# davidfischinger/haf_grasping

Measured on AMD Instinct MI355X. Metric: grid-cell x rotation SVM evals/sec, higher is better.
Workload: dtype f16

## Files before the change

haf_grasping_amd/build.py:

```python
import os
import re
import subprocess
import sys

HERE = os.path.dirname(os.path.abspath(__file__))
CSRC = os.path.join(HERE, "csrc")
LIB = os.path.join(HERE, "libhafgrasp.so")
LIB_TESTING = os.path.join(HERE, "libhafgrasp_testing.so")
ENGINE_SOURCES = ["engine.cpp", "engine_tables.cpp", "engine_request.cpp", "engine_geometry.cpp", "engine_debug.cpp", "engine_topgrasps.cpp"]
TESTING_ONLY = ["engine_testing.cpp", "testkernels.hip"]
SOURCES = ["prestages.hip", "features.hip", "contraction.hip", "screen.hip", "recheck.hip", "exact8.hip", "vote.hip", "prob.hip", "topgrasps.hip"] + \
          ENGINE_SOURCES + ["parsers.cpp", "multi.cpp"]
EXTRA = {"screen.hip": ["-fno-slp-vectorize"]}
HEADERS = ["kernels.h", "device_common.h", "feature_device.h", "screen_band.h", "parsers.h", "decq.h", "engine_internal.h", "engine_state.h"] + TESTING_ONLY + [ os.path.join("..", "..", "include", "hafgrasp.h"),
           os.path.join("..", "cli", "haf_grasp_cli.cpp"), os.path.join("..", "..", "ros_shim", "shim_core.h")]
FLAGS = ["--offload-arch=gfx950", "-O3", "-std=c++17", "-fPIC", "-ffp-contract=off", "-fno-fast-math",
         "-Wall", "-Wno-unused-result", "-Wno-inline-asm"]
ROCM = os.environ.get("ROCM_PATH", "/opt/rocm")
OBJDUMP = os.path.join(ROCM, "lib", "llvm", "bin", "llvm-objdump")
EXP_HAZARD_KERNELS = ["k_svm_screen", "k_svm_rbf_h", "k_svm_rbf"]
EXP_MIN_DISTANCE = 8


def up_to_date():
# ... 117 lines not shown
    for line in text.splitlines():
        m = re.match(r"^[0-9a-f]+ <(\S+)>:", line)
        if m:
            cur = m.group(1) if (DESCRIPTOR_LOAD_KERNELS in m.group(1) and not m.group(1).endswith(".kd")) else None
            if cur:
                rep[cur] = 0
            continue
        if cur and line.split("//")[0].strip().startswith(("global_load", "buffer_load")):
            rep[cur] += 1
    return rep


def check_descriptor_loads(lib=None, verbose=False):
    rep = descriptor_load_report(lib)
    if verbose:
        for k, n in sorted(rep.items()):
            print("  descriptor-load check: %-60s %3d vector loads" % (k[:60], n))
    if not rep:
        raise RuntimeError("check_descriptor_loads: no %s instance found in %s" % (DESCRIPTOR_LOAD_KERNELS, lib or LIB))
    bad = {k: n for k, n in rep.items() if n > MAX_VECTOR_LOADS}
    if bad:
        raise RuntimeError("build check failed: the group-parallel feature kernels fetch descriptor words by vector loads again "
                           "(> %d global/buffer loads): %r" % (MAX_VECTOR_LOADS, bad))
    return rep


READELF = os.path.join(ROCM, "lib", "llvm", "bin", "llvm-readelf")
NO_SPILL_KERNELS = ["k_svm_screen", "k_svm_rbf_h", "k_svm_rbf", "k_recheck_i8"]


def check_no_spills(lib=None, verbose=False):
    import glob
    import shutil
    import tempfile
    lib = lib or LIB
    tmp = tempfile.mkdtemp(prefix="haf_meta_")
    report = {}
    try:
        shutil.copy(lib, os.path.join(tmp, "lib.so"))
        subprocess.check_call([OBJDUMP, "--offloading", "lib.so"], cwd=tmp, stdout=subprocess.DEVNULL)
        for co in sorted(glob.glob(os.path.join(tmp, "*gfx950*"))):
            text = subprocess.check_output([READELF, "--notes", co]).decode(errors="replace")
            name = vg = None
            for line in text.splitlines():
                line = line.strip()
                if line.startswith(".name:"):
# ... 99 lines not shown
```

haf_grasping_amd/capi.py:

```python
import ctypes as C
import os

import numpy as np

HERE = os.path.dirname(os.path.abspath(__file__))
LIB_PATH = os.environ.get("HAF_LIB", os.path.join(HERE, "libhafgrasp.so"))
TESTLIB_PATH = os.environ.get("HAF_TESTLIB", os.path.join(HERE, "libhafgrasp_testing.so"))

HAF_OK, HAF_E_ARG, HAF_E_IO, HAF_E_DEVICE, HAF_E_CAPACITY, HAF_E_BUDGET, HAF_E_INTERNAL = 0, -1, -2, -3, -4, -5, -6
FLAG_KEEP_DEBUG, FLAG_PROFILE, FLAG_FP32_MFMA, FLAG_SPLIT_F16, FLAG_PROBABILITY, FLAG_FULL_RANK = 1, 2, 4, 8, 16, 32
DBG_HEIGHTS, DBG_INTEGRAL, DBG_MASK, DBG_LABELS, DBG_DECISION, DBG_TRANSFORM, DBG_SCREEN_MARGIN, DBG_PROBABILITY, DBG_GRASPSGRID = range(9)
SHARD_ROLLS, SHARD_CLOUDS = 0, 1
STAGES = ["upload", "bin", "integral", "mask", "features", "svm", "refine", "recheck", "vote", "download"]


class Config(C.Structure):
    _fields_ = [("feature_file", C.c_char_p), ("range_file", C.c_char_p), ("model_file", C.c_char_p),
                ("nr_features_without_shaf", C.c_int32), ("grid_h", C.c_int32), ("grid_w", C.c_int32),
                ("n_rolls", C.c_int32), ("roll_step_deg", C.c_int32), ("z_shift", C.c_float),
                ("graspval_top", C.c_int32), ("device", C.c_int32), ("max_clouds", C.c_int32),
                ("max_points", C.c_int64), ("flags", C.c_uint32), ("graspval_th", C.c_int32),
                ("max_rolls_per_call", C.c_int32)]


# ... 121 lines not shown
        L.haf_test_mfma_model.argtypes = [C.c_int, C.c_int, C.c_int, C.POINTER(C.c_double)]
        L.haf_test_scale_device.argtypes = [C.c_void_p, C.c_void_p, C.c_void_p, C.c_double, C.c_double, C.c_void_p,
                                            C.c_int]
        L.haf_test_feature_table.argtypes = [C.c_char_p, C.POINTER(C.c_int), C.c_void_p, C.c_void_p, C.c_int]
        L.haf_test_range_table.argtypes = [C.c_char_p, C.POINTER(C.c_double), C.POINTER(C.c_double),
                                           C.POINTER(C.c_int), C.c_void_p, C.c_void_p, C.c_void_p, C.c_int]
        L.haf_test_model.argtypes = [C.c_char_p, C.POINTER(C.c_double), C.POINTER(C.c_double), C.POINTER(C.c_int),
                                     C.POINTER(C.c_int), C.c_void_p, C.c_void_p, C.c_void_p, C.c_void_p, C.c_long]
        L.haf_test_model_kernel.argtypes = [C.c_char_p, C.POINTER(C.c_int), C.POINTER(C.c_int), C.POINTER(C.c_double), C.POINTER(C.c_double)]
        L.haf_test_roll_geo.argtypes = [C.POINTER(Config), C.POINTER(GraspInput), C.c_int, C.c_void_p, C.c_void_p,
                                        C.c_void_p]
        L.haf_test_finalize.argtypes = [C.POINTER(Config), C.POINTER(GraspInput), C.c_void_p, C.POINTER(GraspOutput)]
        L.haf_test_roll_pose.argtypes = [C.POINTER(Config), C.POINTER(GraspInput), C.c_void_p, C.c_int,
                                         C.POINTER(GraspOutput), C.POINTER(C.c_int32)]
        L.haf_test_mfma_kappa.argtypes = [E, C.c_void_p, C.c_void_p]
        L.haf_test_f16_mfma.argtypes = [C.c_void_p, C.c_void_p, C.c_void_p, C.c_void_p, C.c_int, C.c_int]
        L.haf_test_screen_state.argtypes = [E, C.POINTER(C.c_int), C.POINTER(C.c_int), C.POINTER(C.c_double)]
        L.haf_test_set_screen_inactive.argtypes = [E]
        L.haf_test_check_canaries.argtypes = [C.c_char_p, C.c_int]
        L.haf_test_canary_buffers.argtypes = []
        L.haf_test_poke_flag0_list.argtypes = [E, C.c_int, C.c_int, C.c_int]
        L.haf_test_overflow_stats.argtypes = [E, C.c_void_p]
        L.haf_test_fetch_list.argtypes = [E, C.c_int, C.c_void_p, C.c_int, C.POINTER(C.c_int)]
        L.haf_test_tier_plan.argtypes = [C.c_void_p, C.c_int, C.c_void_p, C.c_int, C.c_int]
        L.haf_test_top_merge.argtypes = [C.POINTER(Config), C.POINTER(GraspInput), C.c_int] + [C.c_void_p] * 5 + \
            [C.c_int, C.c_int, C.c_double, C.c_void_p, C.POINTER(C.c_int32), C.POINTER(C.c_int32)]
    return L


def lib():
    global _lib
    if _lib is None:
        _lib = _bind(LIB_PATH, testing=False)
    return _lib


def multi_plan(devices, shard_mode, n_rolls):
    L = lib()
    n = len(devices)
    dev = (C.c_int32 * max(1, n))(*devices)
    rk, sl, rf, rc_ = [(C.c_int32 * max(1, n))() for _ in range(4)]
    nr = C.c_int32()
    rc = L.haf_multi_plan(dev, n, shard_mode, n_rolls, rk, sl, rf, rc_, C.byref(nr))
    if rc != 0:
        raise HafError(rc, L.haf_multi_last_error(None).decode())
    return dict(rank_of=list(rk)[:n], slot_of=list(sl)[:n], roll_first=list(rf)[:n], roll_count=list(rc_)[:n], n_ranks=nr.value)
# ... 114 lines not shown
        where = 0
        if a.shape[1] == 3:
            for base, nbytes, _ in getattr(self, "_regs", []):
                if base <= a.ctypes.data and a.ctypes.data + a.nbytes <= base + nbytes:
                    where = 2
        return Cloud(a.ctypes.data_as(C.c_void_p), a.shape[0], a.shape[1], where), a

    def model_info(self):
        a, b, c = C.c_int32(), C.c_int32(), C.c_int32()
        self._check(self._L.haf_model_info(self._h, C.byref(a), C.byref(b), C.byref(c)))
        return dict(n_sv=a.value, dim=b.value, n_features=c.value)

    def last_counts(self):
        a, r, b, c = C.c_int64(), C.c_int64(), C.c_int64(), C.c_int64()
        self._check(self._L.haf_last_tiers(self._h, C.byref(a), C.byref(r), C.byref(b), C.byref(c)))
        return dict(n_evals=a.value, n_refined=r.value, n_rechecked=b.value, n_strict=c.value)

    def fetch_list(self, which, cap=1 << 22):
        buf = np.empty(cap, dtype=np.int32)
        n = C.c_int()
        self._check(self._L.haf_test_fetch_list(self._h, which, buf.ctypes.data_as(C.c_void_p), cap, C.byref(n)))
        return buf[:min(n.value, cap)].copy()

    def overflow_stats(self):
        out = (C.c_longlong * 2)()
        self._check(self._L.haf_test_overflow_stats(self._h, out))
        return dict(screening_list_overflows=int(out[0]), extra_windows=int(out[1]))

    def last_exact_tiers(self):
        a, b = C.c_int64(), C.c_int64()
        self._check(self._L.haf_last_exact_tiers(self._h, C.byref(a), C.byref(b)))
        return dict(n_integer=a.value, n_fp64=b.value)

    def last_strict_host(self):
        a = C.c_int64()
        self._check(self._L.haf_last_strict_host(self._h, C.byref(a)))
        return a.value

    def last_prestage(self):
        a = C.c_int64()
        self._check(self._L.haf_last_prestage(self._h, C.byref(a)))
        return dict(n_inexact_grids=a.value)

    def score(self, xyz, grasp_input):
        return self.score_batch([xyz], [grasp_input])[0]

# ... 173 lines not shown
```

haf_grasping_amd/csrc/engine.cpp:

```cpp
#include "engine_state.h"

namespace {

thread_local std::string g_create_error;

}

namespace haf {
static_assert(sizeof(RollRecordDev) == sizeof(haf_roll_record) && sizeof(haf_roll_record) == 16, "roll records travel as 16 bytes");
static_assert(sizeof(AttrRecord) == sizeof(haf_attr_record) && sizeof(haf_attr_record) == 24, "attribute debug record layout");
const void *engine_records_dev(const haf_engine *e) { return e->d_rec.p; }
hipStream_t engine_stream(const haf_engine *e) { return e->stream; }
const haf_config *engine_config(const haf_engine *e) { return &e->cfg; }
void engine_set_error(haf_engine *e, const char *msg) { e->error = msg; }
}

extern "C" {

int haf_abi_version(void) { return HAF_ABI_VERSION; }

void haf_config_default(haf_config *c)
{
    memset(c, 0, sizeof *c);
    c->nr_features_without_shaf = 302;
// ... 12 lines not shown

void haf_grasp_input_default(haf_grasp_input *in)
{
    memset(in, 0, sizeof *in);
    in->grasp_area_length_x = 32;
    in->grasp_area_length_y = 44;
    in->approach_vector[2] = 1.0;
    in->max_calculation_time = 50.0;
    in->gripper_opening_width = 1;
}

const char *haf_last_error(const haf_engine *e) { return e ? e->error.c_str() : g_create_error.c_str(); }

void haf_destroy(haf_engine *e)
{
    if (!e) return;
    if (e->stream) (void)hipStreamSynchronize(e->stream);
    for (auto &r : e->host_regs) (void)hipHostUnregister((void *)r.first);
    e->host_regs.clear();
    e->d_in.release(); e->d_out.release(); e->d_sorted.release(); e->d_bkt.release(); e->d_heights.release(); e->d_rowsum.release(); e->d_inexact.release();
    e->d_ii.release(); e->d_mask.release(); e->d_rowcount.release(); e->d_rowoff.release(); e->d_brcount.release();
    e->d_evalcell.release(); e->d_flag_list.release(); e->d_X.release(); e->d_ax.release();
    e->d_dec.release(); e->d_svt.release(); e->d_svt_h.release(); e->d_labels.release(); e->d_dec_exact.release(); e->d_strict_terms.release(); e->d_part64.release(); e->d_dec_exact2.release(); e->d_flag2_list.release(); e->d_x64.release(); e->d_sv64.release();
    e->d_svt0.release(); e->d_X1.release(); e->d_ax1.release(); e->d_gband.release(); e->d_flag0_list.release(); e->d_flag0_words.release(); e->d_flag0_wgcount.release();
    e->d_own.release(); e->d_gridf.release(); e->d_evf.release(); e->d_ptext.release();
    e->d_sv_i8.release(); e->d_flagi_list.release(); e->d_dec_exacti.release();
    e->d_coef64.release(); e->d_ev16.release(); e->d_attr.release(); e->d_margin.release(); e->d_topkey.release(); e->d_rowmax.release(); e->d_fd.release();
    e->d_sd.release(); e->d_corr.release(); e->d_sd3.release(); e->d_fd_slot.release(); e->d_part1.release();
    e->d_svt_h_cr.release(); e->d_t1_tab.release(); e->d_t1_L.release(); e->d_flag0b_list.release(); e->d_screen_part.release();
    e->d_svt0_cr.release(); e->d_fd_slot_cr.release(); e->d_sd_cr.release(); e->d_sd3_cr.release(); e->d_corr_cr.release();
    e->d_top_scratch.release(); e->d_top_out.release();
    if (e->h_top_out) (void)hipHostFree(e->h_top_out);
    e->d_brslot.release(); e->d_tier_words.release(); e->d_t1_flags.release(); e->d_lr_btiles.release(); e->d_svt_lr.release(); e->d_lr_btiles_in.release(); e->d_corr_lrp.release(); e->d_iiabs.release();
    if (e->h_in) (void)hipHostFree(e->h_in);
    if (e->h_out) (void)hipHostFree(e->h_out);
    for (auto &ev : e->ev) if (ev) (void)hipEventDestroy(ev);
    if (e->own_stream && e->stream) (void)hipStreamDestroy(e->stream);
    delete e;
}
static int calibrate(haf_engine *e)
{
    const haf_config &c = e->cfg;
    if (contraction_mode(c) != MODE_SCREEN || !e->screen_active || e->prob_mode) return HAF_OK;
    const int G = c.grid_h;
    const long cells = (long)G * G;
    const long stride = std::max<long>(1, (cells + c.max_points - 1) / c.max_points);
// ... 389 lines not shown
```

haf_grasping_amd/csrc/engine_request.cpp:

```cpp
#include "engine_state.h"

namespace haf_host {

static double host_kernel_value(const SvmModel &m, const double *xg, int n, int kx)
{
    double acc = 0.0;
    if (m.kernel_type == HAF_KERNEL_RBF) {
        for (int k = 0; k < kx; k++) {
            const double sv = k < m.dim ? m.sv[(size_t)n * m.dim + k] : 0.0;
            const double dd = xg[(size_t)k * 16] - sv;
            acc += dd * dd;
        }
        return std::exp(-m.gamma * acc);
    }
    for (int k = 0; k < kx; k++) {
        const double sv = k < m.dim ? m.sv[(size_t)n * m.dim + k] : 0.0;
        acc += xg[(size_t)k * 16] * sv;
    }
    if (m.kernel_type == HAF_KERNEL_POLY) {
        double tmp = m.gamma * acc + m.coef0, ret = 1.0;
        for (int t = m.degree; t > 0; t /= 2) { if (t % 2 == 1) ret *= tmp; tmp = tmp * tmp; }
        return ret;
    }
    if (m.kernel_type == HAF_KERNEL_SIGMOID) return std::tanh(m.gamma * acc + m.coef0);
// ... 353 lines not shown
    if (q.direct) launch_prob_list(e->d_counters.p, CNT_FLAGGED, e->d_flag_list.p, e->list_cap, s);
    return HAF_OK;
}

static TierFacts tier_facts(const haf_engine *e, const Request &q, int mode, bool reuse_operands)
{
    return TierFacts{e->screen_variant, e->cr_available, e->lr_available, e->lr_enabled, e->lr_plain_available, e->lr_fused,
                     e->use_t0b, e->t1_skip, e->t1_cr_available, e->i8_active, e->calibrated, e->short_gate, e->generic_kernel,
                     e->model.n_sv, test_env("HAF_T0B_NO_GATHER") != nullptr, mode, reuse_operands, q.direct, q.small_exact, q.large,
                     q.fused_pre, (long)q.d.H * q.d.W, q.evals_cap};
}

static void launch_screening(haf_engine *e, const Request &q, const TierPlan &p)
{
    const hipStream_t s = q.s;
    const Dims &d = q.d;
    const long evals_cap = q.evals_cap;
    ScreenParams sp_now = p.sp == SP_LRP ? e->screen_lrp : p.sp == SP_CR ? e->screen_cr : e->screen;
    if (p.sp != SP_LRP) sp_now.cr_poly = e->screen_variant == SCREEN_CR_POLY;
    if (p.lr) { sp_now.lr = 1; sp_now.lr_negflags = e->d_inexact.p; sp_now.lr_iiabs = e->d_iiabs.p; }
    if (!p.reuse)
        launch_features(e->d_ii.p, e->d_evalcell.p, e->d_counters.p, e->d_fd.p, e->d_X.p, e->d_gband.p, d, e->range.lower,
                        e->range.upper, e->svm.neg_gamma2, evals_cap, XMODE_SCREEN, sp_now, nullptr, 0, 0, q.large, q.evals_sel, nullptr, e->d_ax.p, s);
    char *y_img = reinterpret_cast<char *>(e->d_X.p) + (size_t)(e->max_evals_pad / kTile) * (size_t)kS0MatBytes;
    mark(e, HAF_ST_SVM);
    if (p.lr && !e->lr_fused) launch_project(e->d_X.p, e->d_lr_btiles.p, y_img, e->d_gband.p, e->d_counters.p, evals_cap, s);
    if (p.lr)
        launch_svm_screen_lr(e->lr_fused ? reinterpret_cast<char *>(e->d_X.p) : y_img, e->d_gband.p, e->d_ax.p, e->d_svt_lr.p, e->d_evalcell.p, e->d_counters.p, e->svm, e->d_dec.p, e->d_labels.p,
                             e->d_flag0_words.p, e->d_flag0_wgcount.p, list_buf(e, p.pass0_out), e->flag0_cap, e->d_counters.p, d,
                             evals_cap, e->d_margin.p, e->screen_variant, e->crp, e->lr_band, s, handover_counter(p.pass0_out),
                             e->lr_fused ? e->d_lr_btiles_in.p : nullptr);
    else
        launch_svm_screen(e->d_X.p, e->d_gband.p, e->d_ax.p, p.cr ? e->d_svt0_cr.p : e->d_svt0.p, e->d_evalcell.p, e->d_counters.p, e->svm, e->d_dec.p, e->d_labels.p,
                          e->d_flag0_words.p, e->d_flag0_wgcount.p, list_buf(e, p.pass0_out), e->flag0_cap, e->d_counters.p, d, evals_cap, e->d_margin.p,
                          e->screen_variant, e->crp, s, handover_counter(p.pass0_out), nullptr, CNT_EVALS, CNT_FLAGGED0, e->d_screen_part.p, e->screen_parts);
    mark(e, HAF_ST_REFINE);
    const long list_cap = std::min<long>(e->flag0_cap, evals_cap);
    if (p.t0b == T0B_GATHER) {
        launch_svm_screen_lr(reinterpret_cast<char *>(e->d_X.p), e->d_gband.p, e->d_ax.p, e->d_svt_lr.p, e->d_evalcell.p, e->d_counters.p, e->svm, e->d_dec.p,
                             e->d_labels.p, e->d_flag0_words.p, e->d_flag0_wgcount.p, list_buf(e, p.t0b_out), e->flag0_cap,
                             e->d_counters.p, d, list_cap, e->d_margin.p, SCREEN_CR_EXP, e->crp, e->lr_band, s, handover_counter(p.t0b_out),
                             e->d_lr_btiles_in.p, list_buf(e, p.t0b_in), list_counter(p.t0b_in), CNT_FLAGGED0B);
    } else if (p.t0b == T0B_FEATURES) {
        ScreenParams sp_b = e->screen_cr;
        sp_b.cr_poly = 0;
        launch_features(e->d_ii.p, e->d_evalcell.p, e->d_counters.p, e->d_fd.p, e->d_X1.p, e->d_gband.p, d, e->range.lower,
// ... 328 lines not shown
```

haf_grasping_amd/csrc/engine_state.h:

```cpp
#pragma once
#include "../../include/hafgrasp.h"
#include "kernels.h"
#include "parsers.h"
#include "decq.h"
#include "engine_internal.h"

#include <algorithm>
#include <chrono>
#include <cmath>
#include <cstdio>
#include <cstdlib>
#include <cstring>
#include <mutex>
#include <new>
#include <string>
#include <vector>

using namespace haf;

namespace haf_host {

#ifdef HAF_TESTING
inline const char *test_env(const char *name) { return getenv(name); }
#else
// ... 200 lines not shown
    DevBuf<ScrDesc> d_sd;
    DevBuf<ScrCorr> d_corr;
    DevBuf<double> d_part1;
    long part1_stride = 0;
    long large_evals = 1L << 18;
    DevBuf<ScrDesc3> d_sd3;

    RollRecordDev *h_rec = nullptr;
    int *h_counters = nullptr;
    long direct_work = 1L << 21;
    double host_exp_thr = 0.0;
    bool calibrated = false;
    double mfma_kappa = 12.0;
    double mfma_kappa16 = 12.0;
    double mfma_kappa_measured = 0.0, mfma_kappa16_measured = 0.0;
    bool no_bucket_sort = false;
    bool no_fused_pre = false;

    std::vector<std::pair<const char *, size_t>> host_regs;

    long stat_flag0_overflows = 0;
    long stat_extra_windows = 0;
    LastCall last;
    DevBuf<unsigned long long> d_top_scratch;
    DevBuf<char> d_top_out;
    char *h_top_out = nullptr;
    size_t h_top_cap = 0;
};

namespace haf_host {

#define HIPCHK(e, call)                                                                                   \
    do {                                                                                                  \
        hipError_t err__ = (call);                                                                        \
        if (err__ != hipSuccess) {                                                                        \
            (e)->error = std::string(#call) + ": " + hipGetErrorString(err__);                            \
            return HAF_E_DEVICE;                                                                          \
        }                                                                                                 \
    } while (0)

constexpr double kVariantCost[SCREEN_VARIANTS] = {1.0, 1.12, 1.10, 1.16};
constexpr double kUndecidedCost = 8.5;
constexpr double kVariantCostLr[SCREEN_VARIANTS] = {0.80, 1.12, 0.90, 0.87};

constexpr int kShortListGate = 256;
constexpr int kShortGateMinSv = 2048;
// ... 111 lines not shown
```

haf_grasping_amd/csrc/engine_testing.cpp:

```cpp
#include "engine_state.h"

#ifndef HAF_TESTING
#error "engine_testing.cpp belongs to the testing build (-DHAF_TESTING)"
#endif

namespace haf_host {
namespace {
struct CanaryRec { char *user; size_t bytes; const char *file; int line; };
std::mutex g_canary_mu;
std::vector<CanaryRec> g_canary;
}
void canary_register(void *user, size_t bytes, const char *file, int line)
{
    std::lock_guard<std::mutex> lk(g_canary_mu);
    g_canary.push_back(CanaryRec{static_cast<char *>(user), bytes, file, line});
}
void canary_unregister(void *user)
{
    std::lock_guard<std::mutex> lk(g_canary_mu);
    for (size_t i = 0; i < g_canary.size(); i++)
        if (g_canary[i].user == user) { g_canary[i] = g_canary.back(); g_canary.pop_back(); return; }
}
int canary_check(std::string *report)
{
// ... 48 lines not shown
{
    if (!e || !out || !n || cap < 0) return HAF_E_ARG;
    const int *src = nullptr;
    int cnt = 0;
    switch (which) {
        case 0: src = e->d_evalcell.p; cnt = e->last.evals; break;
        case 1: src = e->d_flag_list.p; cnt = std::min(e->last.flagged, e->list_cap); break;
        case 2: src = e->d_flagi_list.p; cnt = e->last.i8 ? std::min(e->last.flaggedi, e->list_cap) : 0; break;
        case 3: src = e->d_flag2_list.p; cnt = std::min(e->last.flagged2, e->list_cap); break;
        case 4: src = e->d_flag0_list.p; cnt = std::min(e->last.flagged0, e->flag0_cap); break;
        default: return HAF_E_ARG;
    }
    *n = cnt;
    if (!src || cnt <= 0) { *n = 0; return HAF_OK; }
    if (hipDeviceSynchronize() != hipSuccess) return HAF_E_DEVICE;
    return hipMemcpy(out, src, (size_t)std::min(cnt, cap) * sizeof(int), hipMemcpyDeviceToHost) == hipSuccess ? HAF_OK : HAF_E_DEVICE;
}
int haf_test_overflow_stats(haf_engine *e, long long *out2)
{
    if (!e || !out2) return HAF_E_ARG;
    out2[0] = e->stat_flag0_overflows; out2[1] = e->stat_extra_windows;
    return HAF_OK;
}
int haf_test_poke_flag0_list(haf_engine *e, int at, int count, int v)
{
    if (!e || !e->d_flag0_list.p) return HAF_E_ARG;
    std::vector<int> h((size_t)count, v);
    return hipMemcpy(e->d_flag0_list.p + e->d_flag0_list.n + at, h.data(), h.size() * sizeof(int), hipMemcpyHostToDevice) == hipSuccess ? HAF_OK : HAF_E_DEVICE;
}

int haf_test_feature_table(const char *path, int *n, int *reg , float *w , int cap)
{
    std::vector<FeatureRow> rows;
    std::string err;
    if (!load_features(path, rows, err)) return HAF_E_IO;
    *n = (int)rows.size();
    for (int i = 0; i < *n && i < cap; i++) {
        memcpy(reg + i * 16, rows[(size_t)i].reg, sizeof rows[0].reg);
        memcpy(w + i * 4, rows[(size_t)i].w, sizeof rows[0].w);
    }
    return HAF_OK;
}

int haf_test_range_table(const char *path, double *lower, double *upper, int *max_index, double *fmin, double *fmax,
                         unsigned char *present, int cap)
{
// ... 296 lines not shown
```

haf_grasping_amd/csrc/feature_device.h:

```cpp
#pragma once
#include "device_common.h"

namespace haf {

typedef __amdgpu_buffer_rsrc_t rsrc_t;
__device__ __forceinline__ rsrc_t make_ii_rsrc(const float *ii, Dims d)
{
    const unsigned bytes = (unsigned)d.B * (unsigned)d.R * (unsigned)((d.H + 1) * (d.W + 1)) * 4u;
    return __builtin_amdgcn_make_buffer_rsrc((void *)ii, 0, (int)bytes, 0x00020000);
}

template <bool UNI>
__device__ __forceinline__ float ii_load(rsrc_t r, unsigned w0b, int off)
{
    if (UNI) return __builtin_bit_cast(float, __builtin_amdgcn_raw_buffer_load_b32(r, (int)w0b, off * 4, 0));
    return __builtin_bit_cast(float, __builtin_amdgcn_raw_buffer_load_b32(r, (int)(w0b + (unsigned)off * 4u), 0, 0));
}

template <bool UNI>
struct SrcBuf {
    rsrc_t r;
    unsigned w0b;
    template <class FD>
    __device__ __forceinline__ float corner(const FD &f, int k, int j) const { return ii_load<UNI>(r, w0b, f.off[k][j]); }
// ... 127 lines not shown
        if (f.active & (1 << k)) {
            const float a = src.corner(f, k, 0), b = src.corner(f, k, 1), c = src.corner(f, k, 2), d = src.corner(f, k, 3);
            const float s1 = __fsub_rn(a, b), s2 = __fsub_rn(s1, c);
            const float R = __fadd_rn(s2, d);
            esum = fmaf(fabsf(f.w[k]), region_round_bound(a, b, c, d, s1, s2, R), esum);
            const float p = __fmul_rn(f.w[k], R);
            ee += fmaf(f.w[k], R, -p);
            rv = __fadd_rn(rv, p);
            if (!first) esum = fmaf(6.1e-8f, fabsf(rv), esum);
            first = false;
        }
    const float q4f = (float)hafq::decq4_float_scr(rv, st);
    nb = f.pad2 * (fabsf(q4f - rv) + fabsf(ee) * 1.000001f + esum + 6.1e-8f * fabsf(rv));
    return fmaf(q4f, (float)f.scr_mul, (float)f.scr_add);
}

constexpr int kBandRows = 15;
constexpr int kBandFloats4 = kBandRows * kBandPitch;

typedef const ScrDesc __attribute__((address_space(4))) *ScrDescK;
__device__ __forceinline__ ScrDescK constant_ptr(const ScrDesc *p) { return (ScrDescK)(unsigned long long)p; }

constexpr float kNbRound = 1.80e-7f, kNbRound3 = 2.40e-7f;
template <int NB>
__device__ __forceinline__ void screen_quad(unsigned band, ScrDescK sd, const hafq::ScrTabs &st, float *ud, float &nu2, float &rmin)
{
    float c[4][8];
    unsigned adr[4][8];
#pragma unroll
    for (int q = 0; q < 4; q++)
#pragma unroll
        for (int j = 0; j < 8; j++) adr[q][j] = band + (unsigned)sd[q].off[j];
#pragma unroll
    for (int q = 0; q < 4; q++)
#pragma unroll
        for (int j = 0; j < 8; j++) {
            const unsigned a = adr[q][j];
            asm volatile("s_mov_b32 m0, %1\n\ts_nop 0\n\tds_read_addtid_b32 %0" : "=v"(c[q][j]) : "s"(a) : "m0");
        }
    asm volatile("s_waitcnt lgkmcnt(0)"
                 : "+v"(c[0][0]), "+v"(c[0][1]), "+v"(c[0][2]), "+v"(c[0][3]), "+v"(c[0][4]), "+v"(c[0][5]), "+v"(c[0][6]), "+v"(c[0][7]));
#pragma unroll
    for (int q = 1; q < 4; q++)
        asm volatile("" : "+v"(c[q][0]), "+v"(c[q][1]), "+v"(c[q][2]), "+v"(c[q][3]), "+v"(c[q][4]), "+v"(c[q][5]), "+v"(c[q][6]),
                          "+v"(c[q][7]));
#pragma unroll
    for (int q = 0; q < 4; q++) {
        const float s10 = __fsub_rn(c[q][0], c[q][1]), s20 = __fsub_rn(s10, c[q][2]), s11 = __fsub_rn(c[q][4], c[q][5]), s21 = __fsub_rn(s11, c[q][6]);
        const float R0 = __fadd_rn(s20, c[q][3]);
        const float R1 = __fadd_rn(s21, c[q][7]);
        const float r0 = __fmul_rn(sd[q].w[0], R0);
        const float r1 = __fmul_rn(sd[q].w[1], R1);
        const float v = __fadd_rn(r0, r1);
        const float q4f = (float)hafq::decq4_float_scr(v, st);
        ud[q] = fmaf(q4f, sd[q].scr_mul, sd[q].scr_add);
        if (NB) {
            float ar = 0.0f;
            if (NB == 2)
                ar = fabsf(sd[q].w[0]) * region_round_bound(c[q][0], c[q][1], c[q][2], c[q][3], s10, s20, R0) +
                     fabsf(sd[q].w[1]) * region_round_bound(c[q][4], c[q][5], c[q][6], c[q][7], s11, s21, R1);
            float nbq = fmaf(kNbRound, fabsf(r0) + fabsf(r1), fabsf(q4f - v));
            if (NB == 2) nbq += ar;
            if (NB == 1) rmin = fminf(fminf(R0, R1), rmin);
            nbq *= sd[q].pad;
            nu2 = fmaf(nbq, nbq, nu2);
            asm volatile("" : "+v"(nu2));
        }
    }
}
__device__ __forceinline__ void screen_quad(unsigned band, ScrDescK sd, const hafq::ScrTabs &st, float *ud) { float dummy = 0.0f, dmin = 0.0f; screen_quad<0>(band, sd, st, ud, dummy, dmin); }

typedef const ScrDesc3 __attribute__((address_space(4))) *ScrDesc3K;
__device__ __forceinline__ ScrDesc3K constant_ptr(const ScrDesc3 *p) { return (ScrDesc3K)(unsigned long long)p; }

template <int NB, int NQ>
__device__ __forceinline__ void screen_pair3(unsigned band, ScrDesc3K sd, const hafq::ScrTabs &st, float *ud, float &nu2, float &rmin)
{
    float c[NQ][12];
    unsigned adr[NQ][12];
#pragma unroll
    for (int q = 0; q < NQ; q++)
#pragma unroll
        for (int j = 0; j < 12; j++) adr[q][j] = band + (unsigned)sd[q].off[j];
#pragma unroll
    for (int q = 0; q < NQ; q++)
#pragma unroll
        for (int j = 0; j < 12; j++) {
            const unsigned a = adr[q][j];
            asm volatile("s_mov_b32 m0, %1\n\ts_nop 0\n\tds_read_addtid_b32 %0" : "=v"(c[q][j]) : "s"(a) : "m0");
        }
    asm volatile("s_waitcnt lgkmcnt(0)"
                 : "+v"(c[0][0]), "+v"(c[0][1]), "+v"(c[0][2]), "+v"(c[0][3]), "+v"(c[0][4]), "+v"(c[0][5]), "+v"(c[0][6]), "+v"(c[0][7]),
                   "+v"(c[0][8]), "+v"(c[0][9]), "+v"(c[0][10]), "+v"(c[0][11]));
    if (NQ > 1)
        asm volatile("" : "+v"(c[NQ - 1][0]), "+v"(c[NQ - 1][1]), "+v"(c[NQ - 1][2]), "+v"(c[NQ - 1][3]), "+v"(c[NQ - 1][4]), "+v"(c[NQ - 1][5]), "+v"(c[NQ - 1][6]), "+v"(c[NQ - 1][7]),
                          "+v"(c[NQ - 1][8]), "+v"(c[NQ - 1][9]), "+v"(c[NQ - 1][10]), "+v"(c[NQ - 1][11]));
#pragma unroll
    for (int q = 0; q < NQ; q++) {
        float r[3], Rk[3], ar = 0.0f;
#pragma unroll
        for (int k = 0; k < 3; k++) {
            const float s1 = __fsub_rn(c[q][4 * k], c[q][4 * k + 1]), s2 = __fsub_rn(s1, c[q][4 * k + 2]);
            Rk[k] = __fadd_rn(s2, c[q][4 * k + 3]);
            r[k] = __fmul_rn(sd[q].w[k], Rk[k]);
            if (NB == 2) ar = fmaf(fabsf(sd[q].w[k]), region_round_bound(c[q][4 * k], c[q][4 * k + 1], c[q][4 * k + 2], c[q][4 * k + 3], s1, s2, Rk[k]), ar);
        }
        float v;
        if (sd[q].shaf) {
            v = -1.0f;
            if (r[1] > r[0] && r[1] > r[2]) {
                const float a = __fsub_rn(r[1], r[0]), b = __fsub_rn(r[1], r[2]);
                v = (b < a) ? b : a;
            }
// ... 45 lines not shown
```

haf_grasping_amd/csrc/features.hip:

```cpp
#include "feature_device.h"

namespace haf {


__device__ __forceinline__ void store_group_img(char *img, int r, int g, half8 v)
{
#define HAF_X_STORE(p, v) __builtin_nontemporal_store(v, p)
    if (g < kHFull * 4) {
        HAF_X_STORE(reinterpret_cast<half8 *>(img + h_image_offset(r, g * 8)), v);
    } else {
        const half4 v0 = {v[0], v[1], v[2], v[3]}, v1 = {v[4], v[5], v[6], v[7]};
        HAF_X_STORE(reinterpret_cast<half4 *>(img + h_image_offset(r, g * 8)), v0);
        HAF_X_STORE(reinterpret_cast<half4 *>(img + h_image_offset(r, g * 8 + 4)), v1);
    }
}
__device__ __forceinline__ void store_group_h(char *xtile, int r, int g, half8 hi, half8 lo)
{
    store_group_img(xtile, r, g, hi);
    store_group_img(xtile + kHMatBytes, r, g, lo);
}

struct ScreenSums { float su2, sd2, cr, ub; };
template <class Corr>
__device__ __forceinline__ _Float16 screen_operand(float ud, ScreenSums &a, const Corr &k)
// ... 260 lines not shown
            for (int g = 0; g < kS0Groups; g++) store_group_img(xtile, r, g, z);
        } else {
            for (int k = 0; k < kKP; k++) xcol[k * kTile] = 0.0f;
        }
        if (MODE == XMODE_SCREEN) { const float zb[kBandFloats] = {0.0f, 0.0f, 0.0f, 0.0f, LR ? __builtin_inff() : 0.0f, 0.0f, 0.0f, 0.0f}; store_band(ax + kBandFloats * e, zb); ax2[e] = 0.0f; }
        else ax[e] = 0.0f;
        return;
    }
    const rsrc_t iir = make_ii_rsrc(ii, d);
    const int e_src = idx_list ? idx_list[e] : (int)e;
    const unsigned w0 = window_origin(evalcell[e_src], d.H, d.W);
    AttrRecord *rec = (MODE != XMODE_SCREEN && dbg) ? dbg + (size_t)e_src * kKP : nullptr;
    double xx = 0.0;
    if (MODE == XMODE_SCREEN) {
        ScreenSums2 acc2{};
        float sx = 0.0f;
        const bool lr_nb = LR && fastwave && lr_exact;
        float nu2 = 0.0f;
        float rmin = 0.0f;
        for (int g = 0; g < kS0Groups; g++) {
            float ud[8];
            if (lr_nb) {
                if ((sp.fast_groups >> g) & 1) {
                    screen_quad<1>(band, constant_ptr(sp.sd) + g * 8, st, ud, nu2, rmin);
                    screen_quad<1>(band, constant_ptr(sp.sd) + g * 8 + 4, st, ud + 4, nu2, rmin);
                } else {
#pragma unroll
                    for (int q = 0; q < 8; q++) screen_pair3<1, 1>(band, constant_ptr(sp.sd3) + g * 8 + q, st, ud + q, nu2, rmin);
                }
            } else if (LR && fastwave) {
                if ((sp.fast_groups >> g) & 1) {
                    screen_quad<2>(band, constant_ptr(sp.sd) + g * 8, st, ud, nu2, rmin);
                    screen_quad<2>(band, constant_ptr(sp.sd) + g * 8 + 4, st, ud + 4, nu2, rmin);
                } else {
#pragma unroll
                    for (int q = 0; q < 8; q++) screen_pair3<2, 1>(band, constant_ptr(sp.sd3) + g * 8 + q, st, ud + q, nu2, rmin);
                }
            } else if (fastwave && ((sp.fast_groups >> g) & 1)) {
                screen_quad(band, constant_ptr(sp.sd) + g * 8, st, ud);
                screen_quad(band, constant_ptr(sp.sd) + g * 8 + 4, st, ud + 4);
            } else if (fastwave) {
#pragma unroll
                for (int q = 0; q < 8; q += 2) screen_pair3(band, constant_ptr(sp.sd3) + g * 8 + q, st, ud + q);
            } else if (LR && !fastwave) {
#pragma unroll
                for (int q = 0; q < 8; q++) {
                    const FeatDesc &F = fd[g * 8 + q];
                    float nbq = 0.0f;
                    ud[q] = F.skip ? 0.0f : screen_attribute_lr(SrcBuf<true>{iir, w0}, F, st, nbq);
                    nu2 = fmaf(nbq, nbq, nu2);
                }
            } else {
#pragma unroll
                for (int q = 0; q < 8; q++) {
                    const FeatDesc &F = fd[g * 8 + q];
                    ud[q] = F.skip ? 0.0f : screen_attribute(SrcBuf<true>{iir, w0}, F, st);
                }
            }
            half8 hi;
#pragma unroll
            for (int q = 0; q < 8; q += 2) {
                const half2v h = screen_operand2(ud[q], ud[q + 1], acc2, constant_ptr(sp.corr2) + g * 4 + (q >> 1));
                hi[q] = h[0]; hi[q + 1] = h[1];
// ... 593 lines not shown
```

Baseline: 532.4 million.

## Software-pipeline screen corner reads with explicit scalar descriptor loads and paired math

Replaces the four-feature screen_quad with a screen_group that processes a group of eight features as four pairs. Scalar descriptor loads for the next pair are issued while the LDS corner reads of the current pair are in flight. Corner reads now compute m0 with s_add_i32 directly from the scalar offset instead of a separately precomputed address, trimming scalar work per read. The per-pair math is written with two-wide float vectors. Adds test-only snapshot buffers and a build-time disassembly audit of slot-loop overhead and in-flight register hazards. The hand-written s_waitcnt placement and register constraints carry a risk of hazards, which the new audit is meant to catch.

```diff
diff --git a/haf_grasping_amd/build.py b/haf_grasping_amd/build.py
--- a/haf_grasping_amd/build.py
+++ b/haf_grasping_amd/build.py
@@ -163,6 +163,140 @@
     if bad:
         raise RuntimeError("build check failed: the group-parallel feature kernels fetch descriptor words by vector loads again "
                            "(> %d global/buffer loads): %r" % (MAX_VECTOR_LOADS, bad))
+    check_slot_loop(lib, verbose=verbose)
+    return rep
+
+
+SLOT_LOOP_KERNEL = "k_features_serialILi2ELb1"
+SLOT_LOOP_AUDITED = ["k_features_serialILi2ELb1", "k_features_serialILi2ELb0"]
+MAX_SLOT_LOOP_OVERHEAD = 4.05
+
+
+def _device_disassembly(lib, extra=()):
+    import glob
+    import shutil
+    import tempfile
+    tmp = tempfile.mkdtemp(prefix="haf_isa_")
+    try:
+        shutil.copy(lib, os.path.join(tmp, "lib.so"))
+        subprocess.check_call([OBJDUMP, "--offloading", "lib.so"], cwd=tmp, stdout=subprocess.DEVNULL)
+        text = ""
+        for co in sorted(glob.glob(os.path.join(tmp, "*gfx950*"))):
+            text += subprocess.check_output([OBJDUMP, "-d"] + list(extra) + [co]).decode(errors="replace")
+    finally:
+        shutil.rmtree(tmp, ignore_errors=True)
+    return text
+
+
+def _all_regs(text):
+    out = set()
+    for m in re.finditer(r"\b([sv])\[(\d+):(\d+)\]|\b([sv])(\d+)\b", text):
+        if m.group(1):
+            out |= {(m.group(1), i) for i in range(int(m.group(2)), int(m.group(3)) + 1)}
+        else:
+            out.add((m.group(4), int(m.group(5))))
+    return out
+
+
+def inflight_violations(code):
+    queue, bad, loads = [], [], 0
+    for i, ins in enumerate(code):
+        op, _, rest = ins.partition(" ")
+        if op.startswith(("s_branch", "s_cbranch", "s_endpgm", "s_setpc")):
+            queue = []
+            continue
+        if op == "s_waitcnt":
+            m = re.search(r"lgkmcnt\((\d+)\)", ins)
+            if m:
+                n = int(m.group(1))
+                lds = [k for k, e in enumerate(queue) if e[0] == "lds"]
+                keep = set(lds[-n:]) if n else set()
+                queue = [e for k, e in enumerate(queue) if (n and e[0] == "smem") or k in keep]
+            continue
+        flying = set().union(*[e[1] for e in queue]) if queue else set()
+        hit = _all_regs(rest) & flying
+        if hit:
+            bad.append((i, ins, sorted(hit)))
+        if op.startswith(("s_load", "s_buffer_load")):
+            queue.append(("smem", _all_regs(rest.split(",")[0])))
+            loads += 1
+        elif op.startswith(("ds_read", "ds_load")):
+            queue.append(("lds", _all_regs(rest.split(",")[0])))
+            loads += 1
+    return loads, bad
+
+
+def slot_loop_report(lib=None):
+    text = _device_disassembly(lib or LIB, ["--symbolize-operands"])
+    kernels, cur, blk = {}, None, None
+    for line in text.splitlines():
+        m = re.match(r"^[0-9a-f]+ <(\S+)>:", line)
+        if m:
+            if re.fullmatch(r"L\d+", m.group(1)):
+                if cur:
+                    blk = []
+                    kernels[cur].append(blk)
+            else:
+                cur = m.group(1) if any(k in m.group(1) for k in SLOT_LOOP_AUDITED) and not m.group(1).endswith(".kd") else None
+                if cur:
+                    blk = []
+                    kernels[cur] = [blk]
+            continue
+        ins = line.split("//")[0].strip()
+        if cur and ins and not ins.endswith(":"):
+            blk.append(ins)
+
+    def cls(op):
+        if op.startswith("s_nop"):
+            return "nop"
+        if op.startswith("s_waitcnt"):
+            return "wait"
+        if op.startswith(("s_load", "s_buffer_load")):
+            return "smem"
+        if op.startswith(("s_branch", "s_cbranch")):
+            return "branch"
+        if op.startswith("s_"):
+            return "salu"
+        if op.startswith("ds_read_addtid"):
+            return "addtid"
+        if op.startswith("ds_"):
+            return "lds"
+        if op.startswith("v_"):
+            return "valu"
+        return "other"
+
+    rep = {"block": {}, "reads": 0, "overhead": None, "inflight": {}}
+    for name, blocks in kernels.items():
+        rep["inflight"][name] = inflight_violations([i for b in blocks for i in b])
+        if SLOT_LOOP_KERNEL not in name:
+            continue
+        for b in blocks:
+            c = {}
+            for ins in b:
+                k = cls(ins.split()[0])
+                c[k] = c.get(k, 0) + 1
+            if c.get("addtid", 0) > rep["reads"]:
+                rep["block"], rep["reads"] = c, c["addtid"]
+    if rep["reads"]:
+        c = rep["block"]
+        rep["overhead"] = (c.get("salu", 0) + c.get("nop", 0) + c.get("wait", 0)) / float(rep["reads"])
+    return rep
+
+
+def check_slot_loop(lib=None, verbose=False):
+    rep = slot_loop_report(lib)
+    if verbose:
+        print("  slot-loop check: %d corner reads, %r -> overhead %s per read" % (rep["reads"], rep["block"], rep["overhead"]))
+        for k, (n, bad) in sorted(rep["inflight"].items()):
+            print("  slot-loop check: %-40s %4d LDS reads / scalar loads, %d touched in flight" % (k[:40], n, len(bad)))
+    if not rep["reads"] or len(rep["inflight"]) != len(SLOT_LOOP_AUDITED):
+        raise RuntimeError("check_slot_loop: %s or its ds_read_addtid_b32 loop not found in %s (kernel renamed?)" % (SLOT_LOOP_KERNEL, lib or LIB))
+    if rep["overhead"] > MAX_SLOT_LOOP_OVERHEAD:
+        raise RuntimeError("build check failed: %.2f scalar-side instructions per corner read in the slot loop of %s (> %.2f): %r"
+                           % (rep["overhead"], SLOT_LOOP_KERNEL, MAX_SLOT_LOOP_OVERHEAD, rep["block"]))
+    bad = {k: v[1][:4] for k, v in rep["inflight"].items() if v[1]}
+    if bad:
+        raise RuntimeError("build check failed: a register of an LDS read or scalar load in flight is touched before its s_waitcnt: %r" % bad)
     return rep
 
 
diff --git a/haf_grasping_amd/capi.py b/haf_grasping_amd/capi.py
--- a/haf_grasping_amd/capi.py
+++ b/haf_grasping_amd/capi.py
@@ -167,6 +167,8 @@
         L.haf_test_poke_flag0_list.argtypes = [E, C.c_int, C.c_int, C.c_int]
         L.haf_test_overflow_stats.argtypes = [E, C.c_void_p]
         L.haf_test_fetch_list.argtypes = [E, C.c_int, C.c_void_p, C.c_int, C.POINTER(C.c_int)]
+        L.haf_test_snapshot_screen.argtypes = [E, C.c_int]
+        L.haf_test_fetch_snapshot.argtypes = [E, C.c_int, C.c_longlong, C.c_void_p, C.c_longlong, C.POINTER(C.c_longlong)]
         L.haf_test_tier_plan.argtypes = [C.c_void_p, C.c_int, C.c_void_p, C.c_int, C.c_int]
         L.haf_test_top_merge.argtypes = [C.POINTER(Config), C.POINTER(GraspInput), C.c_int] + [C.c_void_p] * 5 + \
             [C.c_int, C.c_int, C.c_double, C.c_void_p, C.POINTER(C.c_int32), C.POINTER(C.c_int32)]
@@ -327,6 +329,19 @@
         self._check(self._L.haf_test_fetch_list(self._h, which, buf.ctypes.data_as(C.c_void_p), cap, C.byref(n)))
         return buf[:min(n.value, cap)].copy()
 
+    def snapshot_screen(self, on=True):
+        self._check(self._L.haf_test_snapshot_screen(self._h, 1 if on else 0))
+
+    def fetch_snapshot(self, which, offset=0, nbytes=None):
+        avail = C.c_longlong()
+        self._check(self._L.haf_test_fetch_snapshot(self._h, which, 0, None, 0, C.byref(avail)))
+        if nbytes is None:
+            nbytes = avail.value - offset
+        buf = np.empty(max(0, nbytes), dtype=np.uint8)
+        if nbytes > 0:
+            self._check(self._L.haf_test_fetch_snapshot(self._h, which, offset, buf.ctypes.data_as(C.c_void_p), nbytes, C.byref(avail)))
+        return buf
+
     def overflow_stats(self):
         out = (C.c_longlong * 2)()
         self._check(self._L.haf_test_overflow_stats(self._h, out))
diff --git a/haf_grasping_amd/csrc/engine.cpp b/haf_grasping_amd/csrc/engine.cpp
--- a/haf_grasping_amd/csrc/engine.cpp
+++ b/haf_grasping_amd/csrc/engine.cpp
@@ -58,6 +58,7 @@
     e->d_ii.release(); e->d_mask.release(); e->d_rowcount.release(); e->d_rowoff.release(); e->d_brcount.release();
     e->d_evalcell.release(); e->d_flag_list.release(); e->d_X.release(); e->d_ax.release();
     e->d_dec.release(); e->d_svt.release(); e->d_svt_h.release(); e->d_labels.release(); e->d_dec_exact.release(); e->d_strict_terms.release(); e->d_part64.release(); e->d_dec_exact2.release(); e->d_flag2_list.release(); e->d_x64.release(); e->d_sv64.release();
+    e->snap_X.release(); e->snap_gband.release(); e->snap_ax.release();
     e->d_svt0.release(); e->d_X1.release(); e->d_ax1.release(); e->d_gband.release(); e->d_flag0_list.release(); e->d_flag0_words.release(); e->d_flag0_wgcount.release();
     e->d_own.release(); e->d_gridf.release(); e->d_evf.release(); e->d_ptext.release();
     e->d_sv_i8.release(); e->d_flagi_list.release(); e->d_dec_exacti.release();
diff --git a/haf_grasping_amd/csrc/engine_request.cpp b/haf_grasping_amd/csrc/engine_request.cpp
--- a/haf_grasping_amd/csrc/engine_request.cpp
+++ b/haf_grasping_amd/csrc/engine_request.cpp
@@ -399,6 +399,13 @@
     if (!p.reuse)
         launch_features(e->d_ii.p, e->d_evalcell.p, e->d_counters.p, e->d_fd.p, e->d_X.p, e->d_gband.p, d, e->range.lower,
                         e->range.upper, e->svm.neg_gamma2, evals_cap, XMODE_SCREEN, sp_now, nullptr, 0, 0, q.large, q.evals_sel, nullptr, e->d_ax.p, s);
+    if (e->snap_on && !p.reuse) {
+        const long cap = std::min<long>(evals_cap, e->max_evals_pad);
+        e->snap_cap = cap;
+        (void)hipMemcpyAsync(e->snap_X.p, e->d_X.p, (size_t)((cap + kTile - 1) / kTile) * (size_t)kS0MatBytes, hipMemcpyDeviceToDevice, s);
+        (void)hipMemcpyAsync(e->snap_gband.p, e->d_gband.p, (size_t)cap * kBandFloats * sizeof(float), hipMemcpyDeviceToDevice, s);
+        (void)hipMemcpyAsync(e->snap_ax.p, e->d_ax.p, (size_t)cap * sizeof(float), hipMemcpyDeviceToDevice, s);
+    }
     char *y_img = reinterpret_cast<char *>(e->d_X.p) + (size_t)(e->max_evals_pad / kTile) * (size_t)kS0MatBytes;
     mark(e, HAF_ST_SVM);
     if (p.lr && !e->lr_fused) launch_project(e->d_X.p, e->d_lr_btiles.p, y_img, e->d_gband.p, e->d_counters.p, evals_cap, s);
diff --git a/haf_grasping_amd/csrc/engine_state.h b/haf_grasping_amd/csrc/engine_state.h
--- a/haf_grasping_amd/csrc/engine_state.h
+++ b/haf_grasping_amd/csrc/engine_state.h
@@ -246,6 +246,10 @@
     long stat_flag0_overflows = 0;
     long stat_extra_windows = 0;
     LastCall last;
+    bool snap_on = false;
+    long snap_cap = 0;
+    DevBuf<char> snap_X;
+    DevBuf<float> snap_gband, snap_ax;
     DevBuf<unsigned long long> d_top_scratch;
     DevBuf<char> d_top_out;
     char *h_top_out = nullptr;
diff --git a/haf_grasping_amd/csrc/engine_testing.cpp b/haf_grasping_amd/csrc/engine_testing.cpp
--- a/haf_grasping_amd/csrc/engine_testing.cpp
+++ b/haf_grasping_amd/csrc/engine_testing.cpp
@@ -94,6 +94,30 @@
     out2[0] = e->stat_flag0_overflows; out2[1] = e->stat_extra_windows;
     return HAF_OK;
 }
+int haf_test_snapshot_screen(haf_engine *e, int on)
+{
+    if (!e) return HAF_E_ARG;
+    if (on && !e->snap_X.p) {
+        if (e->snap_X.alloc((size_t)(e->max_evals_pad / kTile) * (size_t)kS0MatBytes) != hipSuccess ||
+            e->snap_gband.alloc((size_t)e->max_evals_pad * kBandFloats) != hipSuccess || e->snap_ax.alloc((size_t)e->max_evals_pad) != hipSuccess)
+            return HAF_E_DEVICE;
+    }
+    e->snap_on = on != 0;
+    if (!on) e->snap_cap = 0;
+    return HAF_OK;
+}
+int haf_test_fetch_snapshot(haf_engine *e, int which, long long offset, void *out, long long bytes, long long *avail)
+{
+    if (!e || !avail || offset < 0 || bytes < 0 || which < 0 || which > 2) return HAF_E_ARG;
+    const char *src = which == 0 ? e->snap_X.p : which == 1 ? reinterpret_cast<const char *>(e->snap_gband.p) : reinterpret_cast<const char *>(e->snap_ax.p);
+    const long long have = which == 0 ? (long long)((e->snap_cap + kTile - 1) / kTile) * kS0MatBytes
+                                      : (long long)e->snap_cap * (which == 1 ? kBandFloats : 1) * (long long)sizeof(float);
+    *avail = src ? have : 0;
+    if (!bytes) return HAF_OK;
+    if (!src || !out || offset + bytes > have) return HAF_E_ARG;
+    if (hipDeviceSynchronize() != hipSuccess) return HAF_E_DEVICE;
+    return hipMemcpy(out, src + offset, (size_t)bytes, hipMemcpyDeviceToHost) == hipSuccess ? HAF_OK : HAF_E_DEVICE;
+}
 int haf_test_poke_flag0_list(haf_engine *e, int at, int count, int v)
 {
     if (!e || !e->d_flag0_list.p) return HAF_E_ARG;
diff --git a/haf_grasping_amd/csrc/feature_device.h b/haf_grasping_amd/csrc/feature_device.h
--- a/haf_grasping_amd/csrc/feature_device.h
+++ b/haf_grasping_amd/csrc/feature_device.h
@@ -173,53 +173,116 @@
 __device__ __forceinline__ ScrDescK constant_ptr(const ScrDesc *p) { return (ScrDescK)(unsigned long long)p; }
 
 constexpr float kNbRound = 1.80e-7f, kNbRound3 = 2.40e-7f;
+#ifdef HAF_SLOT_PAD2
+#define HAF_SLOT_PAD "s_nop 0\n\ts_nop 0\n\t"
+#else
+#define HAF_SLOT_PAD "s_nop 0\n\t"
+#endif
+#define HAF_CORNER_READ(dst, off, band) "s_add_i32 m0, %" #off ", %" #band "\n\t" HAF_SLOT_PAD "ds_read_addtid_b32 %" #dst "\n\t"
+template <class OffK>
+__device__ __forceinline__ void corner_reads8(unsigned band, OffK off, float *c)
+{
+    asm volatile(HAF_CORNER_READ(0, 8, 16) HAF_CORNER_READ(1, 9, 16) HAF_CORNER_READ(2, 10, 16) HAF_CORNER_READ(3, 11, 16)
+                 HAF_CORNER_READ(4, 12, 16) HAF_CORNER_READ(5, 13, 16) HAF_CORNER_READ(6, 14, 16) HAF_CORNER_READ(7, 15, 16)
+                 : "=v"(c[0]), "=v"(c[1]), "=v"(c[2]), "=v"(c[3]), "=v"(c[4]), "=v"(c[5]), "=v"(c[6]), "=v"(c[7])
+                 : "s"(off[0]), "s"(off[1]), "s"(off[2]), "s"(off[3]), "s"(off[4]), "s"(off[5]), "s"(off[6]), "s"(off[7]), "s"(band)
+                 : "m0", "scc");
+}
+template <class OffK>
+__device__ __forceinline__ void corner_reads4(unsigned band, OffK off, float *c)
+{
+    asm volatile(HAF_CORNER_READ(0, 4, 8) HAF_CORNER_READ(1, 5, 8) HAF_CORNER_READ(2, 6, 8) HAF_CORNER_READ(3, 7, 8)
+                 : "=v"(c[0]), "=v"(c[1]), "=v"(c[2]), "=v"(c[3])
+                 : "s"(off[0]), "s"(off[1]), "s"(off[2]), "s"(off[3]), "s"(band)
+                 : "m0", "scc");
+}
+typedef int s_int8 __attribute__((ext_vector_type(8)));
+typedef float s_float4 __attribute__((ext_vector_type(4)));
+struct PairDesc { s_int8 off0, off1; s_float4 k0, k1; float pad0, pad1; };
+static_assert(offsetof(ScrDesc, off) == 0 && offsetof(ScrDesc, w) == 0x20 && offsetof(ScrDesc, scr_mul) == 0x28 && offsetof(ScrDesc, scr_add) == 0x2c &&
+              offsetof(ScrDesc, pad) == 0x34 && sizeof(ScrDesc) == 0x40, "pair_desc_load reads ScrDesc by byte offsets");
+__device__ __forceinline__ void pair_desc_load(ScrDescK sd, PairDesc &d)
+{
+    asm volatile("s_load_dwordx8 %0, %6, 0x0\n\ts_load_dwordx4 %2, %6, 0x20\n\ts_load_dword %4, %6, 0x34\n\t"
+                 "s_load_dwordx8 %1, %6, 0x40\n\ts_load_dwordx4 %3, %6, 0x60\n\ts_load_dword %5, %6, 0x74"
+                 : "=&s"(d.off0), "=&s"(d.off1), "=&s"(d.k0), "=&s"(d.k1), "=&s"(d.pad0), "=&s"(d.pad1) : "s"(sd));
+}
+__device__ __forceinline__ void desc_wait(PairDesc &d)
+{
+    asm volatile("s_waitcnt lgkmcnt(0)" : "+s"(d.off0), "+s"(d.off1), "+s"(d.k0), "+s"(d.k1), "+s"(d.pad0), "+s"(d.pad1));
+}
+__device__ __forceinline__ void pair_wait(float *c, PairDesc &d)
+{
+    asm volatile("s_waitcnt lgkmcnt(0)" : "+v"(c[0]), "+v"(c[1]), "+v"(c[2]), "+v"(c[3]), "+v"(c[4]), "+v"(c[5]), "+v"(c[6]), "+v"(c[7]),
+                                          "+s"(d.off0), "+s"(d.off1), "+s"(d.k0), "+s"(d.k1), "+s"(d.pad0), "+s"(d.pad1));
+    asm volatile("" : "+v"(c[8]), "+v"(c[9]), "+v"(c[10]), "+v"(c[11]), "+v"(c[12]), "+v"(c[13]), "+v"(c[14]), "+v"(c[15]));
+}
+__device__ __forceinline__ void pair_wait(float *c)
+{
+    asm volatile("s_waitcnt lgkmcnt(0)" : "+v"(c[0]), "+v"(c[1]), "+v"(c[2]), "+v"(c[3]), "+v"(c[4]), "+v"(c[5]), "+v"(c[6]), "+v"(c[7]));
+    asm volatile("" : "+v"(c[8]), "+v"(c[9]), "+v"(c[10]), "+v"(c[11]), "+v"(c[12]), "+v"(c[13]), "+v"(c[14]), "+v"(c[15]));
+}
+struct VecOff { s_int8 v; __device__ __forceinline__ int operator[](int j) const { return v[j]; } };
+__device__ __forceinline__ void pair_reads(unsigned band, const PairDesc &d, float *c)
+{
+    corner_reads8(band, VecOff{d.off0}, c);
+    corner_reads8(band, VecOff{d.off1}, c + 8);
+}
 template <int NB>
-__device__ __forceinline__ void screen_quad(unsigned band, ScrDescK sd, const hafq::ScrTabs &st, float *ud, float &nu2, float &rmin)
-{
-    float c[4][8];
-    unsigned adr[4][8];
-#pragma unroll
-    for (int q = 0; q < 4; q++)
-#pragma unroll
-        for (int j = 0; j < 8; j++) adr[q][j] = band + (unsigned)sd[q].off[j];
-#pragma unroll
-    for (int q = 0; q < 4; q++)
-#pragma unroll
-        for (int j = 0; j < 8; j++) {
-            const unsigned a = adr[q][j];
-            asm volatile("s_mov_b32 m0, %1\n\ts_nop 0\n\tds_read_addtid_b32 %0" : "=v"(c[q][j]) : "s"(a) : "m0");
-        }
-    asm volatile("s_waitcnt lgkmcnt(0)"
-                 : "+v"(c[0][0]), "+v"(c[0][1]), "+v"(c[0][2]), "+v"(c[0][3]), "+v"(c[0][4]), "+v"(c[0][5]), "+v"(c[0][6]), "+v"(c[0][7]));
-#pragma unroll
-    for (int q = 1; q < 4; q++)
-        asm volatile("" : "+v"(c[q][0]), "+v"(c[q][1]), "+v"(c[q][2]), "+v"(c[q][3]), "+v"(c[q][4]), "+v"(c[q][5]), "+v"(c[q][6]),
-                          "+v"(c[q][7]));
-#pragma unroll
-    for (int q = 0; q < 4; q++) {
-        const float s10 = __fsub_rn(c[q][0], c[q][1]), s20 = __fsub_rn(s10, c[q][2]), s11 = __fsub_rn(c[q][4], c[q][5]), s21 = __fsub_rn(s11, c[q][6]);
-        const float R0 = __fadd_rn(s20, c[q][3]);
-        const float R1 = __fadd_rn(s21, c[q][7]);
-        const float r0 = __fmul_rn(sd[q].w[0], R0);
-        const float r1 = __fmul_rn(sd[q].w[1], R1);
-        const float v = __fadd_rn(r0, r1);
-        const float q4f = (float)hafq::decq4_float_scr(v, st);
-        ud[q] = fmaf(q4f, sd[q].scr_mul, sd[q].scr_add);
+__device__ __forceinline__ void pair_math(const float *c, const PairDesc &d, const hafq::ScrTabs &st, float *ud, float &nu2, float &rmin)
+{
+    float ar[2] = {0.0f, 0.0f}, q4f[2];
+    typedef float v2f __attribute__((ext_vector_type(2)));
+    const v2f w0 = {d.k0[0], d.k1[0]}, w1 = {d.k0[1], d.k1[1]};
+    const v2f c0 = {c[0], c[8]}, c1 = {c[1], c[9]}, c2 = {c[2], c[10]}, c3 = {c[3], c[11]}, c4 = {c[4], c[12]}, c5 = {c[5], c[13]}, c6 = {c[6], c[14]},
+              c7 = {c[7], c[15]};
+    const v2f s10 = c0 - c1, s20 = s10 - c2, s11 = c4 - c5, s21 = s11 - c6;
+    const v2f R0 = s20 + c3, R1 = s21 + c7;
+    const v2f r0 = w0 * R0, r1 = w1 * R1;
+    const v2f v = r0 + r1;
+    if (NB == 2)
+#pragma unroll
+        for (int i = 0; i < 2; i++)
+            ar[i] = fabsf(w0[i]) * region_round_bound(c0[i], c1[i], c2[i], c3[i], s10[i], s20[i], R0[i]) +
+                    fabsf(w1[i]) * region_round_bound(c4[i], c5[i], c6[i], c7[i], s11[i], s21[i], R1[i]);
+#pragma unroll
+    for (int i = 0; i < 2; i++) q4f[i] = (float)hafq::decq4_float_scr(v[i], st);
+#pragma unroll
+    for (int i = 0; i < 2; i++) {
+        const s_float4 k = i ? d.k1 : d.k0;
+        ud[i] = fmaf(q4f[i], k[2], k[3]);
         if (NB) {
-            float ar = 0.0f;
-            if (NB == 2)
-                ar = fabsf(sd[q].w[0]) * region_round_bound(c[q][0], c[q][1], c[q][2], c[q][3], s10, s20, R0) +
-                     fabsf(sd[q].w[1]) * region_round_bound(c[q][4], c[q][5], c[q][6], c[q][7], s11, s21, R1);
-            float nbq = fmaf(kNbRound, fabsf(r0) + fabsf(r1), fabsf(q4f - v));
-            if (NB == 2) nbq += ar;
-            if (NB == 1) rmin = fminf(fminf(R0, R1), rmin);
-            nbq *= sd[q].pad;
+            float nbq = fmaf(kNbRound, fabsf(r0[i]) + fabsf(r1[i]), fabsf(q4f[i] - v[i]));
+            if (NB == 2) nbq += ar[i];
+            if (NB == 1) rmin = fminf(fminf(R0[i], R1[i]), rmin);
+            nbq *= i ? d.pad1 : d.pad0;
             nu2 = fmaf(nbq, nbq, nu2);
-            asm volatile("" : "+v"(nu2));
-        }
-    }
-}
-__device__ __forceinline__ void screen_quad(unsigned band, ScrDescK sd, const hafq::ScrTabs &st, float *ud) { float dummy = 0.0f, dmin = 0.0f; screen_quad<0>(band, sd, st, ud, dummy, dmin); }
+        }
+    }
+    if (NB) asm volatile("" : "+v"(nu2));
+}
+template <int NB>
+__device__ __forceinline__ void screen_group(unsigned band, ScrDescK sd, const hafq::ScrTabs &st, float *ud, float &nu2, float &rmin)
+{
+    PairDesc d[3];
+    float c[2][16];
+    pair_desc_load(sd, d[0]);
+    desc_wait(d[0]);
+    pair_reads(band, d[0], c[0]);
+    pair_desc_load(sd + 2, d[1]);
+#pragma unroll
+    for (int p = 0; p < 4; p++) {
+        if (p < 3) {
+            pair_wait(c[p & 1], d[(p + 1) % 3]);
+            pair_reads(band, d[(p + 1) % 3], c[(p + 1) & 1]);
+        } else {
+            pair_wait(c[p & 1]);
+        }
+        if (p < 2) pair_desc_load(sd + 2 * (p + 2), d[(p + 2) % 3]);
+        pair_math<NB>(c[p & 1], d[p % 3], st, ud + 2 * p, nu2, rmin);
+    }
+}
+__device__ __forceinline__ void screen_group(unsigned band, ScrDescK sd, const hafq::ScrTabs &st, float *ud) { float dummy = 0.0f, dmin = 0.0f; screen_group<0>(band, sd, st, ud, dummy, dmin); }
 
 typedef const ScrDesc3 __attribute__((address_space(4))) *ScrDesc3K;
 __device__ __forceinline__ ScrDesc3K constant_ptr(const ScrDesc3 *p) { return (ScrDesc3K)(unsigned long long)p; }
@@ -228,18 +291,11 @@
 __device__ __forceinline__ void screen_pair3(unsigned band, ScrDesc3K sd, const hafq::ScrTabs &st, float *ud, float &nu2, float &rmin)
 {
     float c[NQ][12];
-    unsigned adr[NQ][12];
-#pragma unroll
-    for (int q = 0; q < NQ; q++)
-#pragma unroll
-        for (int j = 0; j < 12; j++) adr[q][j] = band + (unsigned)sd[q].off[j];
-#pragma unroll
-    for (int q = 0; q < NQ; q++)
-#pragma unroll
-        for (int j = 0; j < 12; j++) {
-            const unsigned a = adr[q][j];
-            asm volatile("s_mov_b32 m0, %1\n\ts_nop 0\n\tds_read_addtid_b32 %0" : "=v"(c[q][j]) : "s"(a) : "m0");
-        }
+#pragma unroll
+    for (int q = 0; q < NQ; q++) {
+        corner_reads8(band, sd[q].off, c[q]);
+        corner_reads4(band, sd[q].off + 8, c[q] + 8);
+    }
     asm volatile("s_waitcnt lgkmcnt(0)"
                  : "+v"(c[0][0]), "+v"(c[0][1]), "+v"(c[0][2]), "+v"(c[0][3]), "+v"(c[0][4]), "+v"(c[0][5]), "+v"(c[0][6]), "+v"(c[0][7]),
                    "+v"(c[0][8]), "+v"(c[0][9]), "+v"(c[0][10]), "+v"(c[0][11]));
diff --git a/haf_grasping_amd/csrc/features.hip b/haf_grasping_amd/csrc/features.hip
--- a/haf_grasping_amd/csrc/features.hip
+++ b/haf_grasping_amd/csrc/features.hip
@@ -306,23 +306,20 @@
             float ud[8];
             if (lr_nb) {
                 if ((sp.fast_groups >> g) & 1) {
-                    screen_quad<1>(band, constant_ptr(sp.sd) + g * 8, st, ud, nu2, rmin);
-                    screen_quad<1>(band, constant_ptr(sp.sd) + g * 8 + 4, st, ud + 4, nu2, rmin);
+                    screen_group<1>(band, constant_ptr(sp.sd) + g * 8, st, ud, nu2, rmin);
                 } else {
 #pragma unroll
                     for (int q = 0; q < 8; q++) screen_pair3<1, 1>(band, constant_ptr(sp.sd3) + g * 8 + q, st, ud + q, nu2, rmin);
                 }
             } else if (LR && fastwave) {
                 if ((sp.fast_groups >> g) & 1) {
-                    screen_quad<2>(band, constant_ptr(sp.sd) + g * 8, st, ud, nu2, rmin);
-                    screen_quad<2>(band, constant_ptr(sp.sd) + g * 8 + 4, st, ud + 4, nu2, rmin);
+                    screen_group<2>(band, constant_ptr(sp.sd) + g * 8, st, ud, nu2, rmin);
                 } else {
 #pragma unroll
                     for (int q = 0; q < 8; q++) screen_pair3<2, 1>(band, constant_ptr(sp.sd3) + g * 8 + q, st, ud + q, nu2, rmin);
                 }
             } else if (fastwave && ((sp.fast_groups >> g) & 1)) {
-                screen_quad(band, constant_ptr(sp.sd) + g * 8, st, ud);
-                screen_quad(band, constant_ptr(sp.sd) + g * 8 + 4, st, ud + 4);
+                screen_group(band, constant_ptr(sp.sd) + g * 8, st, ud);
             } else if (fastwave) {
 #pragma unroll
                 for (int q = 0; q < 8; q += 2) screen_pair3(band, constant_ptr(sp.sd3) + g * 8 + q, st, ud + q);
```

Result: faster. 540.3 million, median of 6 (+1.5%).
